# SonyCSLParis/audio-metrics

Hardware: AMD Instinct MI355X
Metric: evaluate() embeddings/sec (FAD+KD+PRDC), 2×100k CLAP-512 sets, 1/2/4/8 GPUs (higher is better)
Workload: dtype f32

## Files before the change

audio-metrics_amd/csrc/pairwise.hip:

```cpp
#include "pairwise_common.h"
#include <algorithm>
#include <vector>
#include <cmath>
#include <type_traits>

namespace am {

__global__ void __launch_bounds__(256) row_sqnorm_kernel(const float* __restrict__ X, int64_t N, int64_t ld,
                                                         int D, float* __restrict__ out) {
    const int lane = threadIdx.x & 63;
    const int64_t row = (int64_t)blockIdx.x * 4 + (threadIdx.x >> 6);
    if (row >= N) return;
    const float* x = X + row * ld;
    float acc = 0.f;
    for (int k = lane * 4; k < D; k += 256) {
        const f32x4 v = load_k4(x, k, D);
        acc = fmaf(v.x, v.x, acc);
        acc = fmaf(v.y, v.y, acc);
        acc = fmaf(v.z, v.z, acc);
        acc = fmaf(v.w, v.w, acc);
    }
#pragma unroll
    for (int off = 32; off >= 1; off >>= 1) acc = acc + __shfl_xor(acc, off);
    if (lane == 0) out[row] = acc;
// ... 1320 lines not shown
extern "C" int am_knn_sym_eligible(int64_t N, int D, int k) {
    if (N < 1 || D < 1 || k < 1 || k > AM_MAX_K) return 0;
    return plan_knn(N, N, D, k, true).sym ? 1 : 0;
}

extern "C" int am_knn_list_width(int k) { return (k < 1 || k > AM_MAX_K) ? 0 : kcap_for(k + 1); }

extern "C" size_t am_knn_part_workspace_bytes(int64_t N, int D, int k) {
    if (N < 1 || D < 1 || k < 1 || k > AM_MAX_K) return 0;
    const KnnPlan p = plan_knn(N, N, D, k, true, true);
    Carver c(nullptr, 0);
    KnnBuffers b;
    carve_knn(c, N, N, p, b);
    if (p.sym && knn_fast_enabled(N, D)) carve_knn_fast(c, N, D, p);
    return c.off;
}

static int knn_bounds_impl(const float* X, int64_t N, int64_t ld, int D, int k, int64_t row0, int64_t nrows, float* out_bound_sq,
                           void* ws, size_t ws_bytes, am_stream_t stream, const PreparedSet* prep) {
    int rc;
    if ((rc = check_matrix(X, N, ld, D, "X")) != AM_OK) return rc;
    AM_REQUIRE(out_bound_sq != nullptr, AM_ERR_BAD_ARG, "out_bound_sq is null");
    AM_REQUIRE(k >= 1 && k <= AM_MAX_K, AM_ERR_UNSUPPORTED_K, "nearest_k %d outside [1, %d]", k, AM_MAX_K);
    AM_REQUIRE(row0 >= 0 && nrows >= 1 && row0 + nrows <= N, AM_ERR_BAD_SHAPE, "row range [%lld, +%lld) outside %lld rows",
               (long long)row0, (long long)nrows, (long long)N);
    hipStream_t st = static_cast<hipStream_t>(stream);
    const KnnPlan p = plan_knn(N, N, D, k, true, true);
    AM_REQUIRE(p.sym, AM_ERR_BAD_SHAPE, "the symmetric k-NN path does not apply to %lld x %d (see am_knn_sym_eligible)",
               (long long)N, D);
    Carver c(ws, ws_bytes);
    float* xn = c.take<float>(N);
    float* partial = c.take<float>((size_t)p.pre_chunks * nrows * p.kcap);
    const bool fast = knn_fast_enabled(N, D);
    uint16_t* xb = fast ? c.take<uint16_t>((size_t)N * half_ld(D)) : nullptr;
    unsigned* maxn = fast ? c.take<unsigned>(4) : nullptr;
    AM_REQUIRE(c.ok(), AM_ERR_WORKSPACE, "workspace too small: need %zu bytes, have %zu", c.off, ws_bytes);
    if ((rc = norms_of(prep, X, N, ld, D, xn, st)) != AM_OK) return rc;
    if (fast) {
        AM_HIP_TRY(hipMemsetAsync(maxn, 0, 4 * sizeof(unsigned), st));
        if (prep != nullptr) {
            hipLaunchKernelGGL(prepared_stats_kernel, dim3(1), dim3(64), 0, st, prep->stats, maxn, 0, 2, 3);
        } else {
            if ((rc = launch_to_half(X, N, ld, D, xn, maxn, 0, xb, st)) != AM_OK) return rc;
            AM_HIP_TRY(hipMemcpyAsync(maxn + 3, maxn + 2, sizeof(unsigned), hipMemcpyDeviceToDevice, st));
        }
        const int64_t ldh = half_ld(D) / 2;
        const float* Xb = reinterpret_cast<const float*>(prep != nullptr ? prep->half : xb);
        auto go = [&](auto kcap_tag) -> int {
            constexpr int KC = decltype(kcap_tag)::value;
            int chunks = p.pre_chunks, r2;
            if (p.tile_rows == WIDE_TILE_ROWS && (KC == 6 || KC == 11)) {
                const int64_t samples = ceil_div(ceil_div(N, WIDE_TILE_ROWS), p.pre_stride);
                chunks = std::min(wide_sample_chunks(ceil_div(nrows, WIDE_TILE_ROWS), samples), p.pre_chunks);
                r2 = launch_knn_wide_sample(KC, Xb, N, ldh, xn, (int)ldh, p.pre_stride, chunks, maxn, partial, row0, nrows, st);
            } else {
                r2 = launch_knn_vt<KC, EV_FAST, false>(Xb + row0 * ldh, nrows, ldh, xn + row0, Xb, N, ldh, xn, (int)ldh, p.pre_chunks,
                                                       p.pre_stride, partial, st, maxn);
            }
            if (r2 != AM_OK) return r2;
            hipLaunchKernelGGL(knn_merge_kernel<KC>, dim3((unsigned)ceil_div(nrows, 256)), dim3(256), 0, st, partial, nrows,
                               chunks, k + 1, 1, out_bound_sq, static_cast<const int*>(nullptr));
            hipLaunchKernelGGL(knn_fast_bound_kernel, dim3((unsigned)ceil_div(nrows, 256)), dim3(256), 0, st, out_bound_sq,
                               out_bound_sq, xn + row0, nrows, maxn, fast_c(D));
            AM_LAUNCH_CHECK();
            return AM_OK;
        };
        switch (p.kcap) {
            case 6:  return go(std::integral_constant<int, 6>{});
            case 11: return go(std::integral_constant<int, 11>{});
            case 16: return go(std::integral_constant<int, 16>{});
            default: return go(std::integral_constant<int, 32>{});
        }
    }
    const float* Xr = X + row0 * ld;
    switch (p.kcap) {
        case 6:  return launch_knn<6>(Xr, nrows, ld, xn + row0, X, N, ld, xn, D, k + 1, p.pre_chunks, p.pre_stride, true, partial, out_bound_sq, st);
        case 11: return launch_knn<11>(Xr, nrows, ld, xn + row0, X, N, ld, xn, D, k + 1, p.pre_chunks, p.pre_stride, true, partial, out_bound_sq, st);
        case 16: return launch_knn<16>(Xr, nrows, ld, xn + row0, X, N, ld, xn, D, k + 1, p.pre_chunks, p.pre_stride, true, partial, out_bound_sq, st);
        default: return launch_knn<32>(Xr, nrows, ld, xn + row0, X, N, ld, xn, D, k + 1, p.pre_chunks, p.pre_stride, true, partial, out_bound_sq, st);
    }
}

template <int KCAP>
static int run_knn_part(const float* X, int64_t N, int64_t ld, int D, int k1, int part, int nparts, float* bounds,
                        float* out_lists, const KnnPlan& p, const KnnBuffers& b, hipStream_t st) {
    AM_HIP_TRY(hipMemsetAsync(b.cnt, 0, (size_t)(N + 1) * sizeof(int), st));
    return launch_knn_sym<KCAP>(X, N, ld, b.xn, bounds, D, k1, p.win_tiles, p.nwin, p.per_win, b.partial, b.cand, b.cnt, p.cap,
                                b.wgq, p.qcap, b.wgq_count, b.ov_list, b.ov_count, nullptr, st, part, nparts, out_lists);
}

extern "C" int am_knn_bounds_f32(const float* X, int64_t N, int64_t ld, int D, int k, int64_t row0, int64_t nrows,
                                 float* out_bound_sq, void* ws, size_t ws_bytes, am_stream_t stream) {
    return knn_bounds_impl(X, N, ld, D, k, row0, nrows, out_bound_sq, ws, ws_bytes, stream, nullptr);
}
extern "C" int am_knn_bounds_prepared_f32(const float* X, int64_t N, int64_t ld, int D, const am_prepared_set* prepared, int k,
                                          int64_t row0, int64_t nrows, float* out_bound_sq, void* ws, size_t ws_bytes,
                                          am_stream_t stream) {
    AM_REQUIRE(prepared_ok(prepared), AM_ERR_BAD_ARG, "prepared set has a null member");
    const PreparedSet ps = prepared_of(prepared);
    return knn_bounds_impl(X, N, ld, D, k, row0, nrows, out_bound_sq, ws, ws_bytes, stream, &ps);
}

static int knn_sym_part_impl(const float* X, int64_t N, int64_t ld, int D, int k, int part, int nparts, float* bounds_sq,
                             float* out_lists, void* ws, size_t ws_bytes, am_stream_t stream, const PreparedSet* prep) {
    int rc;
    if ((rc = check_matrix(X, N, ld, D, "X")) != AM_OK) return rc;
    AM_REQUIRE(bounds_sq && out_lists, AM_ERR_BAD_ARG, "null pointer");
// ... 219 lines not shown
```

audio-metrics_amd/csrc/pairwise_common.h:

```cpp
#pragma once
#include "am_common.h"
#include "tile_engine.h"
#include <stdlib.h>

namespace am {

constexpr int EV_DEFAULT = EV_RSRC | EV_FRAGDB | EV_EARLY;
constexpr int WIDE_TILE_ROWS = 256;

#ifdef AM_DEV_KNOBS
static int env_int(const char* name, int dflt) {
    const char* v = getenv(name);
    return v ? atoi(v) : dflt;
}
static int engine_variant() {
    static const int v = env_int("AM_ENGINE_VARIANT", EV_DEFAULT);
    return v;
}
#else
static constexpr int env_int(const char*, int dflt) { return dflt; }
static constexpr int engine_variant() { return EV_DEFAULT; }
#endif

struct WorkItem {
// ... 313 lines not shown
                    marg4[g4] = mg + xn[nt];
                }
                const float tmin = fminf(fminf(tmin4[0], tmin4[1]), fminf(tmin4[2], tmin4[3]));
                const float mmin = fminf(fminf(marg4[0], marg4[1]), fminf(marg4[2], marg4[3]));
                const float pl = fminf(flt[nt], best[nt][KCAP - 1] + fmaf(e2c, xn[nt], e2n));
                if ((lanes_le(tmin, pl) | lanes_le(mmin, mthr)) == 0ull) continue;
#ifdef AM_DEV_KNOBS
                if constexpr (TBX == WIDE_TILE_ROWS) {
                    if (g_wide_dbg & 16) continue;
                }
#endif
#pragma unroll
                for (int g4 = 0; g4 < 4; ++g4) {
                    if ((lanes_le(tmin4[g4], pl) | lanes_le(marg4[g4], mthr)) == 0ull) continue;
#pragma unroll
                    for (int e = 0; e < 4; ++e) {
                        const int reg = g4 * 4 + e;
                        const float u = fmaf(dsc, acc[mt][nt][reg], xn[nt] + yn[g4][e]);
                        const bool own = u <= pl, mir = mirror && u <= tq[g4][e];
                        const unsigned long long sel = lanes_le(u, pl) | (mirror ? lanes_le(u, tq[g4][e]) : 0ull);
                        if (sel != 0ull) {
                            const int below = __builtin_amdgcn_mbcnt_hi((unsigned)(sel >> 32), __builtin_amdgcn_mbcnt_lo((unsigned)sel, 0u));
                            const int slot = wq + below;
                            wq += __popcll(sel);
                            const unsigned j = jbase + mt * 32 + g4 * 8 + e;
#ifdef AM_DEV_KNOBS
                            if (TBX == WIDE_TILE_ROWS && (g_wide_dbg & 32)) continue;
#endif
                            if (own || mir) store_entry(slot, own ? prow[nt] : j, own ? j : prow[nt], own && mir, u);
                        }
                    }
                }
                const float vmin = tmin <= pl ? fmaxf(tmin, 0.f) : INFINITY;
#ifdef AM_DEV_KNOBS
                if (TBX == WIDE_TILE_ROWS && (g_wide_dbg & 64)) continue;
#endif
                if (lanes_lt(vmin, best[nt][KCAP - 1]) != 0ull) list_insert<KCAP>(best[nt], vmin);
            }
        }
    }
};


constexpr int KNN_WIDE_MAX_KCAP = 11;
int64_t wide_grouped_blocks(int64_t row_blocks, int nchunks, int grp_rows);
int launch_cross_wide(bool want_min, unsigned blocks, const float* Rb, int64_t Nr, int64_t ldr, const float* rnorm, const float* rthr,
                      const float* Cb, int64_t Nc, int64_t ldc, const float* cnorm, const float* cthr, int Dh, int nchunks,
                      int grp_rows, const unsigned* maxn, unsigned* rmin_approx, unsigned* row_any, unsigned* row_cover,
                      int32_t* col_count, uint2* wgq, int qcap, int* wgq_count, uint2* items, uint2* ovq, int* ov_count, int ovcap,
                      int* fail, float fc, hipStream_t st);
int launch_cross_wide_sample(const float* Rb, int64_t Nr, int64_t ldr, const float* rnorm, const float* Cb, int64_t Nc, int64_t ldc,
                             const float* cnorm, const float* cthr, int Dh, int stride, int nchunks, const unsigned* maxn,
                             unsigned* row_any, float fc, hipStream_t st);
int launch_knn_wide_sample(int kcap, const float* Xb, int64_t N, int64_t ldh, const float* xnorm, int Dh, int stride, int nchunks,
                           const unsigned* maxn, float* partial, int64_t row0, int64_t nrows, hipStream_t st);
int launch_knn_wide(int kcap, unsigned nwg, const float* Xb, int64_t N, int64_t ldh, const float* xnorm, float* thr, int Dh,
                    int win_tiles, int nwin, int per_win, int k1, const unsigned* maxn, float* partial, int* cnt, int cap,
                    uint2* wgq, float* wgv, int qcap, int* wgq_count, int part, int nparts, float fc, uint2* ovq, float* ovv,
                    unsigned long long* ovn, int ovcap, const int* skip, int* region_counter, hipStream_t st);

bool pstat_supported(int Dh);
bool pstat64_supported(int Dh);
int launch_cross_pstat(bool want_min, unsigned blocks, const float* Rb, int64_t Nr, int64_t ldr, const float* rnorm, const float* rthr,
                       const float* Cb, int64_t Nc, int64_t ldc, const float* cnorm, const float* cthr, int Dh, int nchunks,
                       int grp_rows, const unsigned* maxn, unsigned* rmin_approx, unsigned* row_any, unsigned* row_cover,
                       int32_t* col_count, uint2* wgq, int qcap, int* wgq_count, uint2* items, uint2* ovq, int* ov_count, int ovcap,
                       int* fail, float fc, hipStream_t st);
int launch_knn_pstat(int kcap, unsigned nwg, const float* Xb, int64_t N, int64_t ldh, const float* xnorm, float* thr, int Dh,
                     int win_tiles, int nwin, int per_win, int k1, const unsigned* maxn, float* partial, int* cnt, int cap,
                     uint2* wgq, float* wgv, int qcap, int* wgq_count, int part, int nparts, float fc, uint2* ovq, float* ovv,
                     unsigned long long* ovn, int ovcap, const int* skip, int* region_counter, hipStream_t st);
static inline bool wide_stationary(int Dh) {
    static const int on = env_int("AM_WIDE_STATIONARY", 1);
    return on != 0 && pstat_supported(Dh);
}

}
```

audio-metrics_amd/csrc/pairwise_fast.h:

```cpp
#pragma once

namespace am {

constexpr int EV_FAST = EV_DEFAULT | EV_F16 | EV_LDS;
constexpr int FAST_MAX_DIM = 4096;
constexpr int FAST_MIN_DIM = 1;
constexpr int FAST_DROP_BITS = 0;
static inline int half_drop_bits() {
    static const int n = std::min(std::max(env_int("AM_HALF_DROP_BITS", FAST_DROP_BITS), 0), 6);
    return n;
}
static inline float fast_c(int D) {
    const int n = half_drop_bits();
    const float rest = 1.9073486328125e-06f + 2.98023223876953125e-08f * sqrtf((float)D) + (float)(D + 1) * 4.76837158203125e-07f;
    if (n == 0) return 0.0009765625f + rest;
    const float u = ldexpf(1.f, -(11 - n)) + ldexpf(1.f, -11);
    return 2.f * u + u * u + rest;
}
constexpr int FAST_LDH_ALIGN = 64;

static inline int64_t half_ld(int D) { return (int64_t)(D + FAST_LDH_ALIGN - 1) / FAST_LDH_ALIGN * FAST_LDH_ALIGN; }

__global__ void __launch_bounds__(256) maxabs_bits_kernel(const float* __restrict__ X, int64_t N, int64_t ld, int D,
                                                          unsigned* __restrict__ out) {
// ... 1280 lines not shown
                                                               const float* __restrict__ xnorm, const unsigned* __restrict__ maxn,
                                                               float fc, int* __restrict__ gate, unsigned char* __restrict__ flat_rows) {
    const int64_t i = (int64_t)blockIdx.x * 256 + threadIdx.x;
    bool flat = false;
    if (i < N) {
        float m[KCAP];
#pragma unroll
        for (int s = 0; s < KCAP; ++s) m[s] = partial[i * KCAP + s];
        for (int c = 1; c < nchunks; ++c) {
            const float* src = partial + ((int64_t)c * N + i) * KCAP;
            for (int s = 0; s < KCAP; ++s) list_insert<KCAP>(m, src[s]);
        }
        (void)k1;
        const float band = 2.f * fc * (xnorm[i] + __uint_as_float(maxn[0]));
        flat = m[KCAP - 1] < INFINITY && m[KCAP - 1] - m[1] <= band;
        if (i < N) flat_rows[i] = (flat && m[KCAP - 1] - m[1] <= 0.0625f * band) ? 1 : 0;
    }
    const unsigned long long b = __ballot(flat);
    if ((threadIdx.x & 63) == 0 && b != 0ull) atomicAdd(gate + 2, __popcll(b));
}

__global__ void __launch_bounds__(256) knn_fast_mask_flat_kernel(const unsigned char* __restrict__ flat_rows, const int* __restrict__ gate,
                                                                 float* __restrict__ thr, int* __restrict__ cnt, int64_t N) {
    if (gate[0] != 0) return;
    const int64_t i = (int64_t)blockIdx.x * 256 + threadIdx.x;
    if (i < N && flat_rows[i]) {
        thr[i] = -INFINITY;
        cnt[i] = FAST_ROW_OVERFLOW;
    }
}

__global__ void knn_fast_decide_kernel(int* __restrict__ gate, int64_t N, int k1, int stage, const int* __restrict__ pair_count,
                                       const unsigned* __restrict__ maxn, int* __restrict__ ov_count) {
    if (threadIdx.x != 0 || blockIdx.x != 0) return;
    if (stage == 0) {
        gate[0] = (int64_t)gate[2] * 8 > N ? 1 : 0;
    } else if (stage == 1) {
        const int64_t per_row = N / 160 > (int64_t)(8 * k1 + 16) ? N / 160 : (int64_t)(8 * k1 + 16);
        const bool volume = (int64_t)*pair_count > N * per_row;
        const bool fixups = (int64_t)gate[3] * 8 > N;
        gate[1] = (gate[0] != 0 || volume || fixups || !half_scale_ok(maxn[2])) ? 1 : 0;
    } else if (gate[1] != 0) {
        *ov_count = (int)(N < 0x7fffffff ? N : 0x7fffffff);
    }
}

static bool knn_fast_enabled(int64_t N, int D) {
    static const int on = env_int("AM_KNN_FAST", 1);
    static const int min_rows_env = env_int("AM_KNN_FAST_MIN_ROWS", 0);
    const int64_t min_rows = min_rows_env > 0 ? min_rows_env : (D >= 256 ? 6144 : D >= 128 ? 8192 : D >= 32 ? 12000 : 16384);
    return on != 0 && N >= min_rows && D >= FAST_MIN_DIM && D <= FAST_MAX_DIM && N < ((int64_t)1 << 31);
}

struct KnnFastBuffers {
    uint16_t* xb;
    unsigned* maxn;
    float* wgv;
    unsigned* fidx;
    int *cnt2, *pair_count;
    uint2* ovq;
    float* ovv;
    unsigned long long* ovn;
    int* gate;
    float* xpartial;
    unsigned char* flat_rows;
    KnnFixup fix;
};
constexpr int KNN_FAST_OVCAP = 1 << 22;

static KnnFastBuffers carve_knn_fast(Carver& c, int64_t N, int D, const KnnPlan& p) {
    KnnFastBuffers f;
    f.xb = c.take<uint16_t>((size_t)N * half_ld(D));
    f.maxn = c.take<unsigned>(4);
    f.wgv = c.take<float>((size_t)p.nwg * p.qcap);
    f.fidx = c.take<unsigned>((size_t)N * p.cap);
    f.cnt2 = c.take<int>(N + 2);
    f.pair_count = f.cnt2 ? f.cnt2 + N : nullptr;
    f.ovn = c.take<unsigned long long>(1);
    f.ovq = c.take<uint2>(KNN_FAST_OVCAP);
    f.ovv = c.take<float>(KNN_FAST_OVCAP);
    f.gate = c.take<int>(8);
    f.xpartial = c.take<float>((size_t)choose_chunks(N, N) * N * p.kcap);
    f.flat_rows = c.take<unsigned char>((size_t)N);
    f.fix = carve_knn_fixup(c, N, D, p.kcap);
    return f;
}

static int wide_sample_chunks(int64_t row_blocks, int64_t samples) {
    int chunks = 1;
    int64_t best_cost = INT64_MAX;
    for (int c = 1; c <= 8 && c <= samples; ++c) {
        const int64_t cost = ceil_div(row_blocks * c, 256) * ceil_div(samples, c);
        if (cost < best_cost) {
            best_cost = cost;
            chunks = c;
        }
    }
    return chunks;
}

template <int KCAP>
static int run_knn_fast(const float* X, int64_t N, int64_t ld, int D, int k1, const KnnPlan& p, const KnnBuffers& b,
                        const KnnFastBuffers& f, float* out_r, hipStream_t st, int part = 0, int nparts = 1,
                        const float* bounds_in = nullptr, float* out_lists = nullptr, const PreparedSet* prep = nullptr,
                        const Knn64Hook* h64 = nullptr) {
    int rc;
    const float fc = h64 != nullptr ? fast_c(D) + 1.9073486328125e-06f : fast_c(D);
    const int64_t ldh = half_ld(D) / 2;
    const int Dh = (int)ldh;
    const float* Xb = reinterpret_cast<const float*>(prep != nullptr ? prep->half : f.xb);
    unsigned* maxn = f.maxn;
    float* thr = b.thr;
    static const int gate_on = env_int("AM_KNN_FAST_GATE", 1);
    int* gate = (gate_on != 0 && bounds_in == nullptr && out_lists == nullptr) ? f.gate : nullptr;
    const int* skip_sweep = gate;
    const int* skip_verify = gate != nullptr ? gate + 1 : nullptr;
    if (gate != nullptr) AM_HIP_TRY(hipMemsetAsync(gate, 0, 4 * sizeof(int), st));
    AM_HIP_TRY(hipMemsetAsync(maxn, 0, 4 * sizeof(unsigned), st));
    if (prep != nullptr) {
        hipLaunchKernelGGL(prepared_stats_kernel, dim3(1), dim3(64), 0, st, prep->stats, maxn, 0, 2, 3);
    } else {
        if ((rc = launch_to_half(X, N, ld, D, b.xn, maxn, 0, f.xb, st)) != AM_OK) return rc;
        AM_HIP_TRY(hipMemcpyAsync(maxn + 3, maxn + 2, sizeof(unsigned), hipMemcpyDeviceToDevice, st));
    }
    if (bounds_in != nullptr) {
        hipLaunchKernelGGL(knn_fast_bound_kernel, dim3((unsigned)ceil_div(N, 256)), dim3(256), 0, st, bounds_in, thr, b.xn, N, maxn, fc);
        AM_LAUNCH_CHECK();
    } else {
        int sample_chunks = p.pre_chunks;
        if (p.tile_rows == WIDE_TILE_ROWS) {
            const int64_t rb = ceil_div(N, WIDE_TILE_ROWS), samples = ceil_div(rb, p.pre_stride);
            sample_chunks = wide_sample_chunks(rb, samples);
            if ((rc = launch_knn_wide_sample(KCAP, Xb, N, ldh, b.xn, Dh, p.pre_stride, sample_chunks, maxn, b.partial, 0, N, st)) != AM_OK)
                return rc;
        } else if ((rc = launch_knn_vt<KCAP, EV_FAST, false>(Xb, N, ldh, b.xn, Xb, N, ldh, b.xn, Dh, p.pre_chunks, p.pre_stride,
                                                             b.partial, st, maxn)) != AM_OK) {
            return rc;
        }
        hipLaunchKernelGGL(knn_merge_kernel<KCAP>, dim3((unsigned)ceil_div(N, 256)), dim3(256), 0, st, b.partial, N, sample_chunks,
                           k1, 1, thr, static_cast<const int*>(nullptr));
        if (gate != nullptr) {
            hipLaunchKernelGGL(knn_fast_predict_kernel<KCAP>, dim3((unsigned)ceil_div(N, 256)), dim3(256), 0, st, b.partial, N,
                               sample_chunks, k1, b.xn, maxn, fc, gate, f.flat_rows);
            hipLaunchKernelGGL(knn_fast_decide_kernel, dim3(1), dim3(64), 0, st, gate, N, k1, 0, f.pair_count, maxn, b.ov_count);
        }
        hipLaunchKernelGGL(knn_fast_bound_kernel, dim3((unsigned)ceil_div(N, 256)), dim3(256), 0, st, thr, thr, b.xn, N, maxn, 2.f * fc);
        AM_LAUNCH_CHECK();
    }
    AM_HIP_TRY(hipMemsetAsync(b.cnt, 0, (size_t)(N + 1) * sizeof(int), st));
    AM_HIP_TRY(hipMemsetAsync(f.cnt2, 0, (size_t)(N + 2) * sizeof(int), st));
    if (gate != nullptr) {
        hipLaunchKernelGGL(knn_fast_mask_flat_kernel, dim3((unsigned)ceil_div(N, 256)), dim3(256), 0, st, f.flat_rows, gate, thr, b.cnt, N);
        AM_LAUNCH_CHECK();
    }
    AM_HIP_TRY(hipMemsetAsync(f.ovn, 0, sizeof(unsigned long long), st));
    const unsigned nwg = (unsigned)p.nwg;
    const int64_t nlist = (int64_t)p.nwin * N * KCAP;
    hipLaunchKernelGGL(fill_u32_kernel, dim3((unsigned)ceil_div(nlist, 256)), dim3(256), 0, st,
                       reinterpret_cast<unsigned*>(b.partial), nlist, 0x7f800000u);
    AM_LAUNCH_CHECK();
    {
        AM_HIP_TRY(ensure_dynamic_lds(reinterpret_cast<const void*>(&knn_fast_kernel<KCAP>), (int)PAIRWISE_LDS_BYTES + 16));
    }
    int qcap = p.qcap;
    const int nsub = p.tile_rows == WIDE_TILE_ROWS ? 8 : 4;
    unsigned nregions = nwg;
    int* region_counter = nullptr;
    if (nparts > 1) {
        const int64_t active = std::max<int64_t>(1, sym_active_items(ceil_div(N, p.tile_rows), p.win_tiles, p.nwin, p.per_win, part, nparts));
        const int64_t grown = std::min<int64_t>((int64_t)nwg * qcap / active, 1 << 18) / 16 * 16;
        qcap = (int)std::max<int64_t>(grown, qcap);
        nregions = (unsigned)std::min<int64_t>(active, (int64_t)nwg * p.qcap / qcap);
        region_counter = f.gate + 4;
        AM_HIP_TRY(hipMemsetAsync(region_counter, 0, sizeof(int), st));
        AM_HIP_TRY(hipMemsetAsync(b.wgq_count, 0, (size_t)nregions * (nsub + 1) * sizeof(int), st));
    }
    const int wcap = qcap / (2 * nsub);
    const unsigned nreg = nregions * (unsigned)(nsub + 1);
    static const int ovcap = std::max(0, std::min(env_int("AM_KNN_FAST_OVCAP", KNN_FAST_OVCAP), KNN_FAST_OVCAP));
    clock_begin(AM_KERNEL_KNN, st);
    if (p.tile_rows == WIDE_TILE_ROWS) {
        const auto launch_sweep = wide_stationary(Dh) ? &launch_knn_pstat : &launch_knn_wide;
        if ((rc = launch_sweep(KCAP, nwg, Xb, N, ldh, b.xn, thr, Dh, p.win_tiles, p.nwin, p.per_win, k1, maxn, b.partial, b.cnt,
                                  p.cap, b.wgq, f.wgv, qcap, b.wgq_count, part, nparts, fc, f.ovq, f.ovv, f.ovn, ovcap,
                                  skip_sweep, region_counter, st)) != AM_OK)
            return rc;
    } else {
        hipLaunchKernelGGL(knn_fast_kernel<KCAP>, dim3(nwg), dim3(ENGINE_THREADS), PAIRWISE_LDS_BYTES + 16, st, Xb, N, ldh, b.xn,
                           thr, Dh, p.win_tiles, p.nwin, p.per_win, k1, maxn, b.partial, b.cnt, p.cap, b.wgq, f.wgv, qcap,
                           b.wgq_count, part, nparts, fc, f.ovq, f.ovv, f.ovn, ovcap, skip_sweep, region_counter);
    }
    clock_end(AM_KERNEL_KNN, st);
    AM_LAUNCH_CHECK();
// ... 90 lines not shown
```

audio-metrics_amd/csrc/pairwise_wide.hip:

```cpp
#include "wide_kernels.h"

namespace am {

#ifdef AM_DEV_KNOBS
static unsigned long long* g_trace_dev = nullptr;
static hipError_t set_wide_dev_symbols(hipStream_t st) {
    const int wdbg = env_int("AM_WIDE_DBG", 0), b0 = env_int("AM_WIDE_TRACE_B0", 0);
    hipError_t e = hipMemcpyToSymbolAsync(HIP_SYMBOL(g_wide_dbg), &wdbg, sizeof(int), 0, hipMemcpyHostToDevice, st);
    if (e != hipSuccess) return e;
    e = hipMemcpyToSymbolAsync(HIP_SYMBOL(g_wide_trace_b0), &b0, sizeof(int), 0, hipMemcpyHostToDevice, st);
    if (e != hipSuccess) return e;
    if (env_int("AM_WIDE_TRACE", 0) && g_trace_dev == nullptr) {
        e = hipMalloc(&g_trace_dev, 64 * 2 * 96 * 6 * sizeof(unsigned long long));
        if (e != hipSuccess) return e;
    }
    if (g_trace_dev != nullptr) {
        e = hipMemsetAsync(g_trace_dev, 0, 64 * 2 * 96 * 6 * sizeof(unsigned long long), st);
        if (e != hipSuccess) return e;
    }
    return hipMemcpyToSymbolAsync(HIP_SYMBOL(g_wide_trace), &g_trace_dev, sizeof(g_trace_dev), 0, hipMemcpyHostToDevice, st);
}
}
extern "C" int am_wide_trace_read(unsigned long long* host, size_t count) {
    if (am::g_trace_dev == nullptr) return -1;
// ... 161 lines not shown
                             unsigned* row_any, float fc, hipStream_t st) {
    AM_HIP_TRY(ensure_dynamic_lds(reinterpret_cast<const void*>(&cross_wide_sample_kernel), (int)CROSS_SAMPLE_LDS_BYTES));
    const unsigned blocks = (unsigned)(ceil_div(Nr, WTB) * nchunks);
    hipLaunchKernelGGL(cross_wide_sample_kernel, dim3(blocks), dim3(WTHREADS), CROSS_SAMPLE_LDS_BYTES, st, Rb, Nr, ldr, rnorm, Cb, Nc,
                       ldc, cnorm, cthr, Dh, stride, nchunks, maxn, row_any, fc);
    AM_LAUNCH_CHECK();
    return AM_OK;
}

template <int KCAP>
struct KnnSampleEpilogue {
    const float* qnorm;
    int64_t n;
    float* aux;
    float dsc;
    float xn[2];
    float best[2][KCAP];
    float aux_n;
    const WLane& L;
    __device__ __forceinline__ KnnSampleEpilogue(const WLane& l) : L(l) {}
    __device__ __forceinline__ void aux_issue(int, int64_t qtile) {
        if (L.tid < WTB) {
            const int64_t j = qtile * WTB + L.tid;
            aux_n = j < n ? qnorm[j] : INFINITY;
        }
    }
    __device__ __forceinline__ void aux_commit(int t) {
        if (L.tid < WTB) aux[(t & 1) * WTB + L.tid] = aux_n;
    }
    __device__ __forceinline__ void finish(int t, int64_t, f32x16 (&acc)[4][2]) {
        const float* a = aux + (t & 1) * WTB + L.wm * 128 + L.h * 4;
#pragma unroll
        for (int mt = 0; mt < 4; ++mt) {
            f32x4 yn[4];
#pragma unroll
            for (int g4 = 0; g4 < 4; ++g4) yn[g4] = *reinterpret_cast<const f32x4*>(a + mt * 32 + g4 * 8);
#pragma unroll
            for (int nt = 0; nt < 2; ++nt) {
                float tmin = INFINITY;
#pragma unroll
                for (int reg = 0; reg < 16; ++reg) tmin = fminf(tmin, fmaf(dsc, acc[mt][nt][reg], xn[nt] + yn[reg >> 2][reg & 3]));
                const float v = fmaxf(tmin, 0.f);
                if (__any(v < best[nt][KCAP - 1])) list_insert<KCAP>(best[nt], v);
            }
        }
    }
};


constexpr size_t KNN_SAMPLE_LDS_BYTES = (WENGINE_LDS_WORDS + 4 * WTB) * sizeof(float);

template <int KCAP>
__global__ void __launch_bounds__(WTHREADS, 1)
knn_wide_sample_kernel(const float* __restrict__ Xb, int64_t N, int64_t ldh, const float* __restrict__ xnorm, int Dh, int stride,
                       int nchunks, const unsigned* __restrict__ maxn, float* __restrict__ partial, int64_t row0, int64_t nrows) {
    extern __shared__ __attribute__((aligned(16))) float lds[];
    const WLane L;
    const int64_t T = (N + WTB - 1) / WTB;
    const int64_t samples = (T + stride - 1) / stride;
    const int64_t pb = blockIdx.x / nchunks;
    const int chunk = blockIdx.x % nchunks;
    const int64_t s0 = samples * chunk / nchunks, s1 = samples * (chunk + 1) / nchunks;
    KnnSampleEpilogue<KCAP> epi(L);
    epi.qnorm = xnorm;
    epi.n = N;
    epi.aux = lds + WENGINE_LDS_WORDS;
    epi.dsc = half_unscale(maxn[2], maxn[2]);
#pragma unroll
    for (int nt = 0; nt < 2; ++nt) {
        const int64_t i = row0 + pb * WTB + L.wn * 64 + nt * 32 + L.r;
        epi.xn[nt] = i < N ? xnorm[i] : INFINITY;
#pragma unroll
        for (int s = 0; s < KCAP; ++s) epi.best[nt][s] = INFINITY;
    }
    if (s1 > s0) wide_pipeline(Xb, N, ldh, StridedTiles{s0, stride}, Xb, N, ldh, row0 + pb * WTB, (int)(s1 - s0), Dh, lds, L, epi);
    __syncthreads();
    float* mg = lds;
#pragma unroll
    for (int nt = 0; nt < 2; ++nt) {
        float* dst = mg + ((L.wn * 64 + nt * 32 + L.r) * 4 + (L.wm * 2 + L.h)) * KCAP;
#pragma unroll
        for (int s = 0; s < KCAP; ++s) dst[s] = epi.best[nt][s];
    }
    __syncthreads();
    if (L.tid < WTB) {
        const int64_t i = pb * WTB + L.tid;
        if (i < nrows) {
            const float* src = mg + L.tid * 4 * KCAP;
            float m[KCAP];
#pragma unroll
            for (int s = 0; s < KCAP; ++s) m[s] = src[s];
            for (int s = KCAP; s < 4 * KCAP; ++s) list_insert<KCAP>(m, src[s]);
            float* out = partial + ((int64_t)chunk * nrows + i) * KCAP;
#pragma unroll
            for (int s = 0; s < KCAP; ++s) out[s] = m[s];
        }
    }
}

template <int KCAP>
static int launch_knn_wide_sample_t(const float* Xb, int64_t N, int64_t ldh, const float* xnorm, int Dh, int stride, int nchunks,
                                    const unsigned* maxn, float* partial, int64_t row0, int64_t nrows, hipStream_t st) {
    AM_HIP_TRY(ensure_dynamic_lds(reinterpret_cast<const void*>(&knn_wide_sample_kernel<KCAP>), (int)KNN_SAMPLE_LDS_BYTES));
    const unsigned blocks = (unsigned)(ceil_div(nrows, WTB) * nchunks);
    hipLaunchKernelGGL(knn_wide_sample_kernel<KCAP>, dim3(blocks), dim3(WTHREADS), KNN_SAMPLE_LDS_BYTES, st, Xb, N, ldh, xnorm, Dh, stride,
                       nchunks, maxn, partial, row0, nrows);
    AM_LAUNCH_CHECK();
    return AM_OK;
}

int launch_knn_wide_sample(int kcap, const float* Xb, int64_t N, int64_t ldh, const float* xnorm, int Dh, int stride, int nchunks,
                           const unsigned* maxn, float* partial, int64_t row0, int64_t nrows, hipStream_t st) {
    if (kcap == 6) return launch_knn_wide_sample_t<6>(Xb, N, ldh, xnorm, Dh, stride, nchunks, maxn, partial, row0, nrows, st);
    AM_REQUIRE(kcap == 11, AM_ERR_UNSUPPORTED_K, "the wide sample pass holds lists of 6 or 11 entries (got %d)", kcap);
    return launch_knn_wide_sample_t<11>(Xb, N, ldh, xnorm, Dh, stride, nchunks, maxn, partial, row0, nrows, st);
}

template <int KCAP>
static int launch_knn_wide_t(unsigned nwg, const float* Xb, int64_t N, int64_t ldh, const float* xnorm, float* thr, int Dh,
                             int win_tiles, int nwin, int per_win, int k1, const unsigned* maxn, float* partial, int* cnt, int cap,
                             uint2* wgq, float* wgv, int qcap, int* wgq_count, int part, int nparts, float fc, uint2* ovq,
                             float* ovv, unsigned long long* ovn, int ovcap, const int* skip, int* region_counter, hipStream_t st) {
    AM_HIP_TRY(ensure_dynamic_lds(reinterpret_cast<const void*>(&knn_wide_kernel<KCAP>), (int)KNN_WIDE_LDS_BYTES));
#ifdef AM_DEV_KNOBS
    AM_HIP_TRY(set_wide_dev_symbols(st));
#endif
    hipLaunchKernelGGL(knn_wide_kernel<KCAP>, dim3(nwg), dim3(WTHREADS), KNN_WIDE_LDS_BYTES, st, Xb, N, ldh, xnorm, thr, Dh, win_tiles,
                       nwin, per_win, k1, maxn, partial, cnt, cap, wgq, wgv, qcap, wgq_count, part, nparts, fc, ovq, ovv, ovn, ovcap, skip, region_counter);
    AM_LAUNCH_CHECK();
    return AM_OK;
}

int launch_knn_wide(int kcap, unsigned nwg, const float* Xb, int64_t N, int64_t ldh, const float* xnorm, float* thr, int Dh,
                    int win_tiles, int nwin, int per_win, int k1, const unsigned* maxn, float* partial, int* cnt, int cap,
                    uint2* wgq, float* wgv, int qcap, int* wgq_count, int part, int nparts, float fc, uint2* ovq, float* ovv,
                    unsigned long long* ovn, int ovcap, const int* skip, int* region_counter, hipStream_t st) {
    if (kcap == 6)
        return launch_knn_wide_t<6>(nwg, Xb, N, ldh, xnorm, thr, Dh, win_tiles, nwin, per_win, k1, maxn, partial, cnt, cap, wgq, wgv,
                                    qcap, wgq_count, part, nparts, fc, ovq, ovv, ovn, ovcap, skip, region_counter, st);
    AM_REQUIRE(kcap == 11, AM_ERR_UNSUPPORTED_K, "the wide k-NN sweep holds lists of 6 or 11 entries (got %d)", kcap);
    return launch_knn_wide_t<11>(nwg, Xb, N, ldh, xnorm, thr, Dh, win_tiles, nwin, per_win, k1, maxn, partial, cnt, cap, wgq, wgv,
                                 qcap, wgq_count, part, nparts, fc, ovq, ovv, ovn, ovcap, skip, region_counter, st);
}

}
```

Measured before the change: 8.659 million.

## Seed kNN bounds with hub rows selected by distance to the mean

Adds a hub-selection pipeline. It computes a sampled column mean, scores each row by its squared distance to that mean, and radix-selects the H closest rows outside the strided sample. It then gathers them and runs an extra wide sample pass against those hubs. The extra candidate lists are merged into the initial kNN thresholds, so the bounds are tighter and the later exact pass can prune more work. The cost is a handful of extra kernels, workspace for the scores and hub rows, and an additional GEMM-like pass of H×N.

Result: no change. 8.615 million (-0.5%).

```diff
diff --git a/audio-metrics_amd/csrc/pairwise.hip b/audio-metrics_amd/csrc/pairwise.hip
--- a/audio-metrics_amd/csrc/pairwise.hip
+++ b/audio-metrics_amd/csrc/pairwise.hip
@@ -1396,7 +1396,7 @@
             if (p.tile_rows == WIDE_TILE_ROWS && (KC == 6 || KC == 11)) {
                 const int64_t samples = ceil_div(ceil_div(N, WIDE_TILE_ROWS), p.pre_stride);
                 chunks = std::min(wide_sample_chunks(ceil_div(nrows, WIDE_TILE_ROWS), samples), p.pre_chunks);
-                r2 = launch_knn_wide_sample(KC, Xb, N, ldh, xn, (int)ldh, p.pre_stride, chunks, maxn, partial, row0, nrows, st);
+                r2 = launch_knn_wide_sample(KC, Xb, N, xn, Xb, N, ldh, xn, (int)ldh, p.pre_stride, chunks, maxn, partial, row0, nrows, st);
             } else {
                 r2 = launch_knn_vt<KC, EV_FAST, false>(Xb + row0 * ldh, nrows, ldh, xn + row0, Xb, N, ldh, xn, (int)ldh, p.pre_chunks,
                                                        p.pre_stride, partial, st, maxn);
diff --git a/audio-metrics_amd/csrc/pairwise_common.h b/audio-metrics_amd/csrc/pairwise_common.h
--- a/audio-metrics_amd/csrc/pairwise_common.h
+++ b/audio-metrics_amd/csrc/pairwise_common.h
@@ -389,8 +389,9 @@
 int launch_cross_wide_sample(const float* Rb, int64_t Nr, int64_t ldr, const float* rnorm, const float* Cb, int64_t Nc, int64_t ldc,
                              const float* cnorm, const float* cthr, int Dh, int stride, int nchunks, const unsigned* maxn,
                              unsigned* row_any, float fc, hipStream_t st);
-int launch_knn_wide_sample(int kcap, const float* Xb, int64_t N, int64_t ldh, const float* xnorm, int Dh, int stride, int nchunks,
-                           const unsigned* maxn, float* partial, int64_t row0, int64_t nrows, hipStream_t st);
+int launch_knn_wide_sample(int kcap, const float* Qb, int64_t nq, const float* qnorm, const float* Xb, int64_t N, int64_t ldh,
+                           const float* xnorm, int Dh, int stride, int nchunks, const unsigned* maxn, float* partial, int64_t row0,
+                           int64_t nrows, hipStream_t st);
 int launch_knn_wide(int kcap, unsigned nwg, const float* Xb, int64_t N, int64_t ldh, const float* xnorm, float* thr, int Dh,
                     int win_tiles, int nwin, int per_win, int k1, const unsigned* maxn, float* partial, int* cnt, int cap,
                     uint2* wgq, float* wgv, int qcap, int* wgq_count, int part, int nparts, float fc, uint2* ovq, float* ovv,
diff --git a/audio-metrics_amd/csrc/pairwise_fast.h b/audio-metrics_amd/csrc/pairwise_fast.h
--- a/audio-metrics_amd/csrc/pairwise_fast.h
+++ b/audio-metrics_amd/csrc/pairwise_fast.h
@@ -1356,6 +1356,249 @@
     return on != 0 && N >= min_rows && D >= FAST_MIN_DIM && D <= FAST_MAX_DIM && N < ((int64_t)1 << 31);
 }
 
+constexpr int KNN_HUB_ROWS = 512;
+constexpr int KNN_HUB_MAX_ROWS = 2048;
+constexpr int KNN_HUB_BINS = 2048;
+constexpr int KNN_HUB_BLOCK_ROWS = 4096;
+constexpr int KNN_HUB_SUM_BLOCKS = 256;
+
+static inline int knn_hub_rows() {
+    static const int h = std::min(std::max(env_int("AM_KNN_HUB_ROWS", KNN_HUB_ROWS), 0), KNN_HUB_MAX_ROWS) / 256 * 256;
+    return h;
+}
+
+__device__ __forceinline__ float half_lo(unsigned w) { return (float)__builtin_bit_cast(_Float16, (unsigned short)(w & 0xffffu)); }
+__device__ __forceinline__ float half_hi(unsigned w) { return (float)__builtin_bit_cast(_Float16, (unsigned short)(w >> 16)); }
+
+__global__ void __launch_bounds__(256) knn_hub_colsum_kernel(const uint4* __restrict__ Xb, int64_t nsel, int64_t step, int Dh,
+                                                             float* __restrict__ part) {
+    __shared__ float red[256][9];
+    const int W4 = Dh / 4, w0 = blockIdx.y * 256;
+    const int W = min(256, W4 - w0), R = 256 / W;
+    const int rsub = threadIdx.x / W, wl = threadIdx.x % W;
+    float a[8] = {0.f, 0.f, 0.f, 0.f, 0.f, 0.f, 0.f, 0.f};
+    if (rsub < R) {
+        const int64_t stride = (int64_t)gridDim.x * R;
+#pragma unroll 4
+        for (int64_t j = (int64_t)blockIdx.x * R + rsub; j < nsel; j += stride) {
+            const uint4 v = Xb[j * step * W4 + w0 + wl];
+            a[0] += half_lo(v.x); a[1] += half_hi(v.x);
+            a[2] += half_lo(v.y); a[3] += half_hi(v.y);
+            a[4] += half_lo(v.z); a[5] += half_hi(v.z);
+            a[6] += half_lo(v.w); a[7] += half_hi(v.w);
+        }
+    }
+#pragma unroll
+    for (int e = 0; e < 8; ++e) red[threadIdx.x][e] = a[e];
+    __syncthreads();
+    if (rsub == 0) {
+        for (int r = 1; r < R; ++r)
+#pragma unroll
+            for (int e = 0; e < 8; ++e) a[e] += red[r * W + wl][e];
+        float* out = part + ((int64_t)blockIdx.x * W4 + w0 + wl) * 8;
+#pragma unroll
+        for (int e = 0; e < 8; ++e) out[e] = a[e];
+    }
+}
+
+__global__ void __launch_bounds__(256) knn_hub_mean_kernel(const float* __restrict__ part, int nblocks, int Dh, int64_t nsel,
+                                                           float* __restrict__ mu, unsigned* __restrict__ hist) {
+    __shared__ float red[4][64];
+    for (int i = blockIdx.x * 256 + threadIdx.x; i < 3 * KNN_HUB_BINS; i += gridDim.x * 256) hist[i] = 0u;
+    const int c = blockIdx.x * 64 + (threadIdx.x & 63), q = threadIdx.x >> 6;
+    float s = 0.f;
+    if (c < 2 * Dh) {
+#pragma unroll 4
+        for (int g = q; g < nblocks; g += 4) s += part[(int64_t)g * 2 * Dh + c];
+    }
+    red[q][threadIdx.x & 63] = s;
+    __syncthreads();
+    if (q == 0 && c < 2 * Dh) mu[c] = (red[0][threadIdx.x] + red[1][threadIdx.x] + red[2][threadIdx.x] + red[3][threadIdx.x]) / (float)nsel;
+}
+
+__device__ __forceinline__ unsigned hub_key(float v) {
+    const unsigned u = __float_as_uint(v);
+    return (u & 0x80000000u) ? ~u : (u | 0x80000000u);
+}
+__device__ __forceinline__ bool hub_eligible(int64_t i, int stride) { return (i / WIDE_TILE_ROWS) % stride != 0; }
+__device__ __forceinline__ int hub_shift(int pass) { return pass == 0 ? 21 : pass == 1 ? 10 : 0; }
+
+__global__ void __launch_bounds__(256) knn_hub_score_kernel(const uint4* __restrict__ Xb, int64_t N, int Dh, const float* __restrict__ mu,
+                                                            const float* __restrict__ xnorm, const unsigned* __restrict__ maxn,
+                                                            float* __restrict__ score, int stride, unsigned* __restrict__ hist) {
+    __shared__ unsigned h[KNN_HUB_BINS];
+    for (int b = threadIdx.x; b < KNN_HUB_BINS; b += 256) h[b] = 0u;
+    __syncthreads();
+    const int lane = threadIdx.x & 63, W4 = Dh / 4;
+    const float dsc = half_unscale(maxn[2], maxn[2]);
+    for (int64_t row = (int64_t)blockIdx.x * 4 + (threadIdx.x >> 6); row < N; row += (int64_t)gridDim.x * 4) {
+        float dot = 0.f;
+        for (int w = lane; w < W4; w += 64) {
+            const uint4 v = Xb[row * W4 + w];
+            const f32x4 m0 = *reinterpret_cast<const f32x4*>(mu + 8 * w), m1 = *reinterpret_cast<const f32x4*>(mu + 8 * w + 4);
+            dot = fmaf(half_lo(v.x), m0.x, fmaf(half_hi(v.x), m0.y, dot));
+            dot = fmaf(half_lo(v.y), m0.z, fmaf(half_hi(v.y), m0.w, dot));
+            dot = fmaf(half_lo(v.z), m1.x, fmaf(half_hi(v.z), m1.y, dot));
+            dot = fmaf(half_lo(v.w), m1.z, fmaf(half_hi(v.w), m1.w, dot));
+        }
+#pragma unroll
+        for (int off = 32; off >= 1; off >>= 1) dot += __shfl_xor(dot, off);
+        if (lane == 0) {
+            const float v = fmaf(dsc, dot, xnorm[row]);
+            score[row] = v;
+            if (hub_eligible(row, stride)) atomicAdd(&h[hub_key(v) >> 21], 1u);
+        }
+    }
+    __syncthreads();
+    for (int b = threadIdx.x; b < KNN_HUB_BINS; b += 256)
+        if (h[b] != 0u) atomicAdd(hist + b, h[b]);
+}
+
+__device__ __forceinline__ void hub_resolve(const unsigned* __restrict__ hist, int passes, unsigned H, unsigned* grp, unsigned* sel) {
+    if (threadIdx.x == 0) {
+        sel[0] = 0u;
+        sel[1] = H;
+    }
+    for (int q = 0; q < passes; ++q) {
+        const unsigned* h = hist + q * KNN_HUB_BINS;
+        unsigned s = 0;
+        for (int b = 0; b < 8; ++b) s += h[threadIdx.x * 8 + b];
+        grp[threadIdx.x] = s;
+        __syncthreads();
+        if (threadIdx.x == 0) {
+            unsigned need = sel[1], g = 0, b = 0;
+            while (g < 255 && grp[g] < need) need -= grp[g++];
+            b = g * 8;
+            while (b < g * 8 + 7 && h[b] < need) need -= h[b++];
+            sel[0] |= b << hub_shift(q);
+            sel[1] = need;
+        }
+        __syncthreads();
+    }
+    __syncthreads();
+}
+
+__global__ void __launch_bounds__(256) knn_hub_hist_kernel(const float* __restrict__ score, int64_t N, int stride, unsigned H,
+                                                           unsigned* __restrict__ hist, int pass) {
+    __shared__ unsigned h[KNN_HUB_BINS];
+    __shared__ unsigned grp[256], sel[2];
+    hub_resolve(hist, pass, H, grp, sel);
+    for (int b = threadIdx.x; b < KNN_HUB_BINS; b += 256) h[b] = 0u;
+    __syncthreads();
+    const int shift = hub_shift(pass), up = pass == 0 ? 32 : hub_shift(pass - 1);
+    const unsigned prefix = sel[0];
+    for (int r = 0; r < KNN_HUB_BLOCK_ROWS / 256; ++r) {
+        const int64_t i = (int64_t)blockIdx.x * KNN_HUB_BLOCK_ROWS + r * 256 + threadIdx.x;
+        if (i < N && hub_eligible(i, stride)) {
+            const unsigned key = hub_key(score[i]);
+            if (up == 32 || (key >> up) == (prefix >> up)) atomicAdd(&h[(key >> shift) & (pass == 2 ? 1023u : 2047u)], 1u);
+        }
+    }
+    __syncthreads();
+    for (int b = threadIdx.x; b < KNN_HUB_BINS; b += 256)
+        if (h[b] != 0u) atomicAdd(hist + pass * KNN_HUB_BINS + b, h[b]);
+}
+
+__global__ void __launch_bounds__(256) knn_hub_count_kernel(const float* __restrict__ score, int64_t N, int stride, unsigned H,
+                                                            const unsigned* __restrict__ hist, uint2* __restrict__ block_count) {
+    __shared__ unsigned grp[256], sel[2], cnt[2];
+    hub_resolve(hist, 3, H, grp, sel);
+    if (threadIdx.x < 2) cnt[threadIdx.x] = 0u;
+    __syncthreads();
+    const unsigned T = sel[0];
+    unsigned less = 0, eq = 0;
+    for (int r = 0; r < KNN_HUB_BLOCK_ROWS / 256; ++r) {
+        const int64_t i = (int64_t)blockIdx.x * KNN_HUB_BLOCK_ROWS + r * 256 + threadIdx.x;
+        if (i < N && hub_eligible(i, stride)) {
+            const unsigned key = hub_key(score[i]);
+            less += key < T;
+            eq += key == T;
+        }
+    }
+    atomicAdd(&cnt[0], less);
+    atomicAdd(&cnt[1], eq);
+    __syncthreads();
+    if (threadIdx.x == 0) block_count[blockIdx.x] = make_uint2(cnt[0], cnt[1]);
+}
+
+__global__ void __launch_bounds__(256) knn_hub_compact_kernel(const float* __restrict__ score, int64_t N, int stride, unsigned H,
+                                                              const unsigned* __restrict__ hist, const uint2* __restrict__ block_count,
+                                                              int* __restrict__ hub_idx) {
+    __shared__ unsigned grp[256], sel[2], base[2], wsum[4];
+    hub_resolve(hist, 3, H, grp, sel);
+    if (threadIdx.x < 2) base[threadIdx.x] = 0u;
+    __syncthreads();
+    unsigned less = 0, eq = 0;
+    for (unsigned b = threadIdx.x; b < blockIdx.x; b += 256) {
+        const uint2 c = block_count[b];
+        less += c.x;
+        eq += c.y;
+    }
+    if (less != 0u) atomicAdd(&base[0], less);
+    if (eq != 0u) atomicAdd(&base[1], eq);
+    __syncthreads();
+    const unsigned T = sel[0], need = sel[1];
+    unsigned less_before = base[0], eq_before = base[1];
+    const int lane = threadIdx.x & 63, wave = threadIdx.x >> 6;
+    for (int r = 0; r < KNN_HUB_BLOCK_ROWS / 256; ++r) {
+        const int64_t i = (int64_t)blockIdx.x * KNN_HUB_BLOCK_ROWS + r * 256 + threadIdx.x;
+        bool is_less = false, is_eq = false;
+        if (i < N && hub_eligible(i, stride)) {
+            const unsigned key = hub_key(score[i]);
+            is_less = key < T;
+            is_eq = key == T;
+        }
+        const unsigned long long bl = __ballot(is_less), be = __ballot(is_eq);
+        const unsigned long long below = (1ull << lane) - 1ull;
+        if (lane == 0) wsum[wave] = (unsigned)__popcll(bl) | ((unsigned)__popcll(be) << 16);
+        __syncthreads();
+        unsigned lb = less_before + (unsigned)__popcll(bl & below), eb = eq_before + (unsigned)__popcll(be & below);
+        unsigned tl = 0, te = 0;
+        for (int w = 0; w < 4; ++w) {
+            const unsigned v = wsum[w];
+            if (w < wave) {
+                lb += v & 0xffffu;
+                eb += v >> 16;
+            }
+            tl += v & 0xffffu;
+            te += v >> 16;
+        }
+        if (is_less || (is_eq && eb < need)) {
+            const unsigned pos = lb + min(eb, need);
+            if (pos < H) hub_idx[pos] = (int)i;
+        }
+        less_before += tl;
+        eq_before += te;
+        __syncthreads();
+    }
+}
+
+__global__ void __launch_bounds__(256) knn_hub_gather_kernel(const unsigned* __restrict__ Xb, int64_t N, int Dh, const float* __restrict__ xnorm,
+                                                             const int* __restrict__ hub_idx, int H, unsigned* __restrict__ rows,
+                                                             float* __restrict__ norms) {
+    const int lane = threadIdx.x & 63;
+    const int j = blockIdx.x * 4 + (threadIdx.x >> 6);
+    if (j >= H) return;
+    const int64_t i = hub_idx[j];
+    const bool ok = i >= 0 && i < N;
+    for (int w = lane; w < Dh; w += 64) rows[(int64_t)j * Dh + w] = ok ? Xb[i * Dh + w] : 0u;
+    if (lane == 0) norms[j] = ok ? xnorm[i] : INFINITY;
+}
+
+struct KnnHubBuffers {
+    float *colpart, *mu, *score, *norm;
+    unsigned* hist;
+    uint2* block_count;
+    int* idx;
+    uint16_t* rows;
+};
+
+static int64_t knn_hub_eligible_rows(int64_t N, int stride) {
+    int64_t strided = 0;
+    for (int64_t t = 0; t * WIDE_TILE_ROWS < N; t += stride) strided += std::min<int64_t>(WIDE_TILE_ROWS, N - t * WIDE_TILE_ROWS);
+    return N - strided;
+}
+
 struct KnnFastBuffers {
     uint16_t* xb;
     unsigned* maxn;
@@ -1369,6 +1612,7 @@
     float* xpartial;
     unsigned char* flat_rows;
     KnnFixup fix;
+    KnnHubBuffers hub;
 };
 constexpr int KNN_FAST_OVCAP = 1 << 22;
 
@@ -1387,6 +1631,18 @@
     f.xpartial = c.take<float>((size_t)choose_chunks(N, N) * N * p.kcap);
     f.flat_rows = c.take<unsigned char>((size_t)N);
     f.fix = carve_knn_fixup(c, N, D, p.kcap);
+    f.hub = KnnHubBuffers{};
+    if (p.tile_rows == WIDE_TILE_ROWS && knn_hub_rows() > 0) {
+        const size_t H = (size_t)knn_hub_rows(), ldw = (size_t)half_ld(D);
+        f.hub.colpart = c.take<float>((size_t)KNN_HUB_SUM_BLOCKS * ldw);
+        f.hub.mu = c.take<float>(ldw);
+        f.hub.score = c.take<float>((size_t)N);
+        f.hub.norm = c.take<float>(H);
+        f.hub.hist = c.take<unsigned>(3 * KNN_HUB_BINS);
+        f.hub.block_count = c.take<uint2>((size_t)ceil_div(N, KNN_HUB_BLOCK_ROWS));
+        f.hub.idx = c.take<int>(H);
+        f.hub.rows = c.take<uint16_t>(H * ldw);
+    }
     return f;
 }
 
@@ -1401,6 +1657,33 @@
         }
     }
     return chunks;
+}
+
+static int run_knn_hub_sample(int kcap, const float* Xb, int64_t N, int64_t ldh, const float* xn, int Dh, int stride, int H, int chunks,
+                              const unsigned* maxn, const KnnHubBuffers& hb, float* partial, hipStream_t st) {
+    const unsigned* Xw = reinterpret_cast<const unsigned*>(Xb);
+    const uint4* X4 = reinterpret_cast<const uint4*>(Xb);
+    const int64_t step = std::max<int64_t>(1, N / 16384), nsel = ceil_div(N, step);
+    const int rows_at_once = 256 / std::min(256, Dh / 4);
+    const int sum_blocks = (int)std::min<int64_t>(KNN_HUB_SUM_BLOCKS, ceil_div(nsel, (int64_t)rows_at_once * 4));
+    const unsigned sel_blocks = (unsigned)ceil_div(N, KNN_HUB_BLOCK_ROWS);
+    hipLaunchKernelGGL(knn_hub_colsum_kernel, dim3((unsigned)sum_blocks, (unsigned)ceil_div(Dh / 4, 256)), dim3(256), 0, st, X4, nsel, step,
+                       Dh, hb.colpart);
+    hipLaunchKernelGGL(knn_hub_mean_kernel, dim3((unsigned)ceil_div(2 * Dh, 64)), dim3(256), 0, st, hb.colpart, sum_blocks, Dh, nsel, hb.mu,
+                       hb.hist);
+    hipLaunchKernelGGL(knn_hub_score_kernel, dim3((unsigned)std::min<int64_t>(ceil_div(N, 4), 4096)), dim3(256), 0, st, X4, N, Dh, hb.mu,
+                       xn, maxn, hb.score, stride, hb.hist);
+    AM_LAUNCH_CHECK();
+    for (int pass = 1; pass < 3; ++pass)
+        hipLaunchKernelGGL(knn_hub_hist_kernel, dim3(sel_blocks), dim3(256), 0, st, hb.score, N, stride, (unsigned)H, hb.hist, pass);
+    hipLaunchKernelGGL(knn_hub_count_kernel, dim3(sel_blocks), dim3(256), 0, st, hb.score, N, stride, (unsigned)H, hb.hist, hb.block_count);
+    hipLaunchKernelGGL(knn_hub_compact_kernel, dim3(sel_blocks), dim3(256), 0, st, hb.score, N, stride, (unsigned)H, hb.hist,
+                       hb.block_count, hb.idx);
+    hipLaunchKernelGGL(knn_hub_gather_kernel, dim3((unsigned)ceil_div(H, 4)), dim3(256), 0, st, Xw, N, Dh, xn, hb.idx, H,
+                       reinterpret_cast<unsigned*>(hb.rows), hb.norm);
+    AM_LAUNCH_CHECK();
+    return launch_knn_wide_sample(kcap, reinterpret_cast<const float*>(hb.rows), H, hb.norm, Xb, N, ldh, xn, Dh, 1, chunks, maxn,
+                                  partial, 0, N, st);
 }
 
 template <int KCAP>
@@ -1431,18 +1714,28 @@
         hipLaunchKernelGGL(knn_fast_bound_kernel, dim3((unsigned)ceil_div(N, 256)), dim3(256), 0, st, bounds_in, thr, b.xn, N, maxn, fc);
         AM_LAUNCH_CHECK();
     } else {
-        int sample_chunks = p.pre_chunks;
+        int sample_chunks = p.pre_chunks, merge_chunks = 0;
         if (p.tile_rows == WIDE_TILE_ROWS) {
             const int64_t rb = ceil_div(N, WIDE_TILE_ROWS), samples = ceil_div(rb, p.pre_stride);
             sample_chunks = wide_sample_chunks(rb, samples);
-            if ((rc = launch_knn_wide_sample(KCAP, Xb, N, ldh, b.xn, Dh, p.pre_stride, sample_chunks, maxn, b.partial, 0, N, st)) != AM_OK)
+            if ((rc = launch_knn_wide_sample(KCAP, Xb, N, b.xn, Xb, N, ldh, b.xn, Dh, p.pre_stride, sample_chunks, maxn, b.partial, 0, N,
+                                             st)) != AM_OK)
                 return rc;
+            const int room = std::max(p.nchunks, p.pre_chunks) - sample_chunks;
+            const int64_t H = std::min<int64_t>(knn_hub_rows(), knn_hub_eligible_rows(N, p.pre_stride));
+            if (H > 0 && room > 0 && f.hub.rows != nullptr) {
+                const int chunks = std::min(wide_sample_chunks(rb, ceil_div(H, WIDE_TILE_ROWS)), room);
+                if ((rc = run_knn_hub_sample(KCAP, Xb, N, ldh, b.xn, Dh, p.pre_stride, (int)H, chunks, maxn, f.hub,
+                                             b.partial + (size_t)sample_chunks * N * KCAP, st)) != AM_OK)
+                    return rc;
+                merge_chunks = sample_chunks + chunks;
+            }
         } else if ((rc = launch_knn_vt<KCAP, EV_FAST, false>(Xb, N, ldh, b.xn, Xb, N, ldh, b.xn, Dh, p.pre_chunks, p.pre_stride,
                                                              b.partial, st, maxn)) != AM_OK) {
             return rc;
         }
-        hipLaunchKernelGGL(knn_merge_kernel<KCAP>, dim3((unsigned)ceil_div(N, 256)), dim3(256), 0, st, b.partial, N, sample_chunks,
-                           k1, 1, thr, static_cast<const int*>(nullptr));
+        hipLaunchKernelGGL(knn_merge_kernel<KCAP>, dim3((unsigned)ceil_div(N, 256)), dim3(256), 0, st, b.partial, N,
+                           std::max(merge_chunks, sample_chunks), k1, 1, thr, static_cast<const int*>(nullptr));
         if (gate != nullptr) {
             hipLaunchKernelGGL(knn_fast_predict_kernel<KCAP>, dim3((unsigned)ceil_div(N, 256)), dim3(256), 0, st, b.partial, N,
                                sample_chunks, k1, b.xn, maxn, fc, gate, f.flat_rows);
diff --git a/audio-metrics_amd/csrc/pairwise_wide.hip b/audio-metrics_amd/csrc/pairwise_wide.hip
--- a/audio-metrics_amd/csrc/pairwise_wide.hip
+++ b/audio-metrics_amd/csrc/pairwise_wide.hip
@@ -237,18 +237,19 @@
 
 template <int KCAP>
 __global__ void __launch_bounds__(WTHREADS, 1)
-knn_wide_sample_kernel(const float* __restrict__ Xb, int64_t N, int64_t ldh, const float* __restrict__ xnorm, int Dh, int stride,
-                       int nchunks, const unsigned* __restrict__ maxn, float* __restrict__ partial, int64_t row0, int64_t nrows) {
+knn_wide_sample_kernel(const float* __restrict__ Qb, int64_t nq, const float* __restrict__ qnorm, const float* __restrict__ Xb,
+                       int64_t N, int64_t ldh, const float* __restrict__ xnorm, int Dh, int stride, int nchunks,
+                       const unsigned* __restrict__ maxn, float* __restrict__ partial, int64_t row0, int64_t nrows) {
     extern __shared__ __attribute__((aligned(16))) float lds[];
     const WLane L;
-    const int64_t T = (N + WTB - 1) / WTB;
+    const int64_t T = (nq + WTB - 1) / WTB;
     const int64_t samples = (T + stride - 1) / stride;
     const int64_t pb = blockIdx.x / nchunks;
     const int chunk = blockIdx.x % nchunks;
     const int64_t s0 = samples * chunk / nchunks, s1 = samples * (chunk + 1) / nchunks;
     KnnSampleEpilogue<KCAP> epi(L);
-    epi.qnorm = xnorm;
-    epi.n = N;
+    epi.qnorm = qnorm;
+    epi.n = nq;
     epi.aux = lds + WENGINE_LDS_WORDS;
     epi.dsc = half_unscale(maxn[2], maxn[2]);
 #pragma unroll
@@ -258,7 +259,7 @@
 #pragma unroll
         for (int s = 0; s < KCAP; ++s) epi.best[nt][s] = INFINITY;
     }
-    if (s1 > s0) wide_pipeline(Xb, N, ldh, StridedTiles{s0, stride}, Xb, N, ldh, row0 + pb * WTB, (int)(s1 - s0), Dh, lds, L, epi);
+    if (s1 > s0) wide_pipeline(Qb, nq, ldh, StridedTiles{s0, stride}, Xb, N, ldh, row0 + pb * WTB, (int)(s1 - s0), Dh, lds, L, epi);
     __syncthreads();
     float* mg = lds;
 #pragma unroll
@@ -284,21 +285,23 @@
 }
 
 template <int KCAP>
-static int launch_knn_wide_sample_t(const float* Xb, int64_t N, int64_t ldh, const float* xnorm, int Dh, int stride, int nchunks,
-                                    const unsigned* maxn, float* partial, int64_t row0, int64_t nrows, hipStream_t st) {
+static int launch_knn_wide_sample_t(const float* Qb, int64_t nq, const float* qnorm, const float* Xb, int64_t N, int64_t ldh,
+                                    const float* xnorm, int Dh, int stride, int nchunks, const unsigned* maxn, float* partial,
+                                    int64_t row0, int64_t nrows, hipStream_t st) {
     AM_HIP_TRY(ensure_dynamic_lds(reinterpret_cast<const void*>(&knn_wide_sample_kernel<KCAP>), (int)KNN_SAMPLE_LDS_BYTES));
     const unsigned blocks = (unsigned)(ceil_div(nrows, WTB) * nchunks);
-    hipLaunchKernelGGL(knn_wide_sample_kernel<KCAP>, dim3(blocks), dim3(WTHREADS), KNN_SAMPLE_LDS_BYTES, st, Xb, N, ldh, xnorm, Dh, stride,
-                       nchunks, maxn, partial, row0, nrows);
+    hipLaunchKernelGGL(knn_wide_sample_kernel<KCAP>, dim3(blocks), dim3(WTHREADS), KNN_SAMPLE_LDS_BYTES, st, Qb, nq, qnorm, Xb, N, ldh,
+                       xnorm, Dh, stride, nchunks, maxn, partial, row0, nrows);
     AM_LAUNCH_CHECK();
     return AM_OK;
 }
 
-int launch_knn_wide_sample(int kcap, const float* Xb, int64_t N, int64_t ldh, const float* xnorm, int Dh, int stride, int nchunks,
-                           const unsigned* maxn, float* partial, int64_t row0, int64_t nrows, hipStream_t st) {
-    if (kcap == 6) return launch_knn_wide_sample_t<6>(Xb, N, ldh, xnorm, Dh, stride, nchunks, maxn, partial, row0, nrows, st);
+int launch_knn_wide_sample(int kcap, const float* Qb, int64_t nq, const float* qnorm, const float* Xb, int64_t N, int64_t ldh,
+                           const float* xnorm, int Dh, int stride, int nchunks, const unsigned* maxn, float* partial, int64_t row0,
+                           int64_t nrows, hipStream_t st) {
+    if (kcap == 6) return launch_knn_wide_sample_t<6>(Qb, nq, qnorm, Xb, N, ldh, xnorm, Dh, stride, nchunks, maxn, partial, row0, nrows, st);
     AM_REQUIRE(kcap == 11, AM_ERR_UNSUPPORTED_K, "the wide sample pass holds lists of 6 or 11 entries (got %d)", kcap);
-    return launch_knn_wide_sample_t<11>(Xb, N, ldh, xnorm, Dh, stride, nchunks, maxn, partial, row0, nrows, st);
+    return launch_knn_wide_sample_t<11>(Qb, nq, qnorm, Xb, N, ldh, xnorm, Dh, stride, nchunks, maxn, partial, row0, nrows, st);
 }
 
 template <int KCAP>
```
